# Yotsuei/ClearConverse

Hardware: AMD Instinct MI355X
Metric: xRT (audio-sec/wall-sec) end-to-end, 30 s 16 kHz clips (higher is better)
Workload: dtype bf16

## Files before the change

### clearconverse_amd/csrc/resnet.hip

```cpp
#include <string>
#include <vector>
#include <math.h>
#include "../../include/ccx.h"
#include "ccx_common.h"
#include "gemm_bf16.h"
#include "model_store.h"

namespace {

constexpr int FB_LEN = 400, FB_SHIFT = 160, FB_NFFT = 512, FB_MELS = 80, FB_MELW = 64;
constexpr int RN_C0 = 32, RN_EMB = 256, RN_STAGES = 4;
constexpr int RN_BLOCKS[RN_STAGES] = {3, 4, 6, 3};

__global__ __launch_bounds__(256) void fbank_kernel(const float* __restrict__ wav, long stride, int T, const float* __restrict__ window,
                                                    const float2* __restrict__ twiddle, const float* __restrict__ melw,
                                                    const int* __restrict__ mel_start, const int* __restrict__ mel_len,
                                                    float* __restrict__ feats_t) {
  __shared__ float2 buf[4][FB_NFFT];
  __shared__ float2 tw[FB_NFFT / 2];
  const int lane = threadIdx.x & 63, wave = threadIdx.x >> 6;
  for (int i = threadIdx.x; i < FB_NFFT / 2; i += 256) tw[i] = twiddle[i];
  const int chunk = blockIdx.y;
  const int t = blockIdx.x * 4 + wave;
  const bool live = t < T;
  const float* x = wav + (long)chunk * stride + (long)(live ? t : 0) * FB_SHIFT;
  float2* b = buf[wave];
  float v[7];
  float sm = 0.f;
#pragma unroll
  for (int j = 0; j < 7; j++) {
    const int i = lane + 64 * j;
    v[j] = i < FB_LEN ? x[i] * 32768.f : 0.f;
    sm += v[j];
  }
  const float mean = wave_reduce_sum(sm) / (float)FB_LEN;
#pragma unroll
  for (int j = 0; j < 7; j++) {
    const int i = lane + 64 * j;
    if (i < FB_LEN) b[i].y = v[j] - mean;
  }
  __syncthreads();
  float z[7];
#pragma unroll
  for (int j = 0; j < 7; j++) {
    const int i = lane + 64 * j;
    z[j] = 0.f;
    if (i < FB_LEN) z[j] = (b[i].y - 0.97f * b[i > 0 ? i - 1 : 0].y) * window[i];
  }
  __syncthreads();
#pragma unroll
  for (int j = 0; j < 8; j++) {
    const int i = lane + 64 * j;
    const int r = (int)(__brev((unsigned)i) >> 23);
    b[r] = make_float2(j < 7 ? z[j] : 0.f, 0.f);
  }
  __syncthreads();
  for (int s = 1; s <= 9; s++) {
    const int half = 1 << (s - 1);
#pragma unroll
    for (int q = 0; q < 4; q++) {
      const int bf = lane + 64 * q;
      const int grp = bf >> (s - 1), pos = bf & (half - 1);
      const int i0 = (grp << s) + pos, i1 = i0 + half;
      const float2 w = tw[pos << (9 - s)];
      const float2 a = b[i0], c = b[i1];
      const float2 m = make_float2(c.x * w.x - c.y * w.y, c.x * w.y + c.y * w.x);
      b[i0] = make_float2(a.x + m.x, a.y + m.y);
      b[i1] = make_float2(a.x - m.x, a.y - m.y);
    }
    __syncthreads();
  }
#pragma unroll
  for (int q = 0; q < 4; q++) {
    const int k = lane + 64 * q;
    const float2 c = b[k];
    b[k].x = c.x * c.x + c.y * c.y;
  }
  __syncthreads();
  for (int m = lane; m < FB_MELS; m += 64) {
    const int st = mel_start[m], ln = mel_len[m];
    float acc = 0.f;
    for (int k = 0; k < ln; k++) acc = fmaf(melw[m * FB_MELW + k], b[st + k].x, acc);
    if (live) feats_t[((long)chunk * FB_MELS + m) * T + t] = logf(fmaxf(acc, 1.1920929e-07f));
  }
}

__global__ __launch_bounds__(256) void fbank_mean_kernel(const float* __restrict__ feats_t, int T, float* __restrict__ mean) {
  __shared__ float sh[4];
  const float* p = feats_t + (long)blockIdx.x * T;
  float s = 0.f;
  for (int i = threadIdx.x; i < T; i += 256) s += p[i];
  s = wave_reduce_sum(s);
  if ((threadIdx.x & 63) == 0) sh[threadIdx.x >> 6] = s;
  __syncthreads();
  if (threadIdx.x == 0) mean[blockIdx.x] = (sh[0] + sh[1] + sh[2] + sh[3]) / (float)T;
}

__global__ __launch_bounds__(256) void conv1_kernel(const float* __restrict__ feats_t, const float* __restrict__ mean, int T,
                                                    const float* __restrict__ w, const float* __restrict__ bias,
                                                    bf16_t* __restrict__ out) {
  __shared__ float sw[RN_C0 * 9 + RN_C0];
  for (int i = threadIdx.x; i < RN_C0 * 9 + RN_C0; i += 256) sw[i] = i < RN_C0 * 9 ? w[i] : bias[i - RN_C0 * 9];
  __syncthreads();
  const int t = blockIdx.x * 256 + threadIdx.x;
  const int f = blockIdx.y, chunk = blockIdx.z;
  if (t >= T) return;
  float x[9];
#pragma unroll
  for (int kh = 0; kh < 3; kh++) {
    const int ff = f + kh - 1;
    const bool fin = ff >= 0 && ff < FB_MELS;
    const float mu = fin ? mean[chunk * FB_MELS + ff] : 0.f;
    const float* row = feats_t + ((long)chunk * FB_MELS + (fin ? ff : 0)) * T;
#pragma unroll
    for (int kw = 0; kw < 3; kw++) {
      const int tt = t + kw - 1;
      x[kh * 3 + kw] = (fin && tt >= 0 && tt < T) ? row[tt] - mu : 0.f;
    }
  }
  const long Wp = T + 2;
  bf16_t* dst = out + (((long)chunk * (FB_MELS + 2) + f + 1) * Wp + t + 1) * RN_C0;
#pragma unroll
  for (int c8 = 0; c8 < RN_C0 / 8; c8++) {
    float o[8];
#pragma unroll
    for (int j = 0; j < 8; j++) {
      const int c = c8 * 8 + j;
      float a = sw[RN_C0 * 9 + c];
#pragma unroll
      for (int k = 0; k < 9; k++) a = fmaf(sw[c * 9 + k], x[k], a);
      o[j] = fmaxf(a, 0.f);
    }
    uint4 pk;
    pk.x = pack_bf16x2(o[0], o[1]); pk.y = pack_bf16x2(o[2], o[3]); pk.z = pack_bf16x2(o[4], o[5]); pk.w = pack_bf16x2(o[6], o[7]);
    ((uint4*)dst)[c8] = pk;
  }
}

template <bool HAS_RESID>
__global__ __launch_bounds__(256) void conv3x3_c32_kernel(const bf16_t* __restrict__ in, const bf16_t* __restrict__ wpk,
                                                          const float* __restrict__ bias, const bf16_t* __restrict__ resid,
                                                          bf16_t* __restrict__ out, int H, int W) {
  constexpr int TW = 64, TH = 4, PITCH = 96;
  __shared__ __attribute__((aligned(16))) char tile[(TH + 2) * (TW + 2) * PITCH];
  const int tid = threadIdx.x, lane = tid & 63, wave = tid >> 6;
  const int l15 = lane & 15, hq = lane >> 4;
  const long Wp = W + 2;
  const int y0 = blockIdx.y * TH, img = blockIdx.z;
  const bf16_t* src = in + ((long)img * (H + 2) + y0) * Wp * 32;
  constexpr int NCH = (TH + 2) * (TW + 2) * 4, NIT = (NCH + 255) / 256;
  uint4 stg[NIT];
  uint4 rres[4];
  const long orow = ((long)img * (H + 2) + y0 + wave + 1) * Wp + 1;
  auto fetch = [&](int x0) {
#pragma unroll
    for (int it = 0; it < NIT; it++) {
      const int idx = tid + 256 * it;
      const int row = idx / ((TW + 2) * 4), rem = idx - row * (TW + 2) * 4;
      const int px = rem >> 2, q = rem & 3;
      stg[it] = make_uint4(0, 0, 0, 0);
      if (idx < NCH && x0 + px < Wp) stg[it] = *(const uint4*)(src + ((long)row * Wp + x0 + px) * 32 + q * 8);
    }
    if (HAS_RESID) {
#pragma unroll
      for (int pt = 0; pt < 4; pt++) {
        const int x = x0 + pt * 16 + l15;
        rres[pt] = make_uint4(0, 0, 0, 0);
        if (x < W) rres[pt] = *(const uint4*)(resid + (orow + x) * 32 + 8 * hq);
      }
    }
  };
  auto put = [&]() {
#pragma unroll
    for (int it = 0; it < NIT; it++) {
      const int idx = tid + 256 * it;
      const int row = idx / ((TW + 2) * 4), rem = idx - row * (TW + 2) * 4;
      const int px = rem >> 2, q = rem & 3;
      if (idx < NCH) *(uint4*)(tile + (row * (TW + 2) + px) * PITCH + q * 16) = stg[it];
    }
  };
  fetch(0);
  bf16x8 wf[9][2];
#pragma unroll
  for (int t = 0; t < 9; t++)
#pragma unroll
    for (int j = 0; j < 2; j++) {
      const int co = 8 * (l15 >> 2) + 4 * j + (l15 & 3);
      wf[t][j] = *(const bf16x8*)(wpk + (long)co * 384 + (t / 3) * 128 + (t % 3) * 32 + hq * 8);
    }
  float bv[8];
#pragma unroll
  for (int i = 0; i < 8; i++) bv[i] = bias[8 * hq + i];
  const int n_tiles = (W + TW - 1) / TW;
  for (int k = 0; k < n_tiles; k++) {
    const int x0 = k * TW;
    put();
    uint4 rcur[4];
    if (HAS_RESID) {
#pragma unroll
      for (int pt = 0; pt < 4; pt++) rcur[pt] = rres[pt];
    }
    __syncthreads();
    if (k + 1 < n_tiles) fetch(x0 + TW);
    f32x4 acc[4][2];
#pragma unroll
    for (int pt = 0; pt < 4; pt++)
#pragma unroll
      for (int j = 0; j < 2; j++) acc[pt][j] = (f32x4){0.f, 0.f, 0.f, 0.f};
#pragma unroll
    for (int t = 0; t < 9; t++) {
      const int kh = t / 3, kw = t % 3;
#pragma unroll
      for (int pt = 0; pt < 4; pt++) {
        const bf16x8 bfrag = *(const bf16x8*)(tile + ((wave + kh) * (TW + 2) + pt * 16 + l15 + kw) * PITCH + hq * 16);
#pragma unroll
        for (int j = 0; j < 2; j++) acc[pt][j] = __builtin_amdgcn_mfma_f32_16x16x32_bf16(wf[t][j], bfrag, acc[pt][j], 0, 0, 0);
      }
    }
#pragma unroll
    for (int pt = 0; pt < 4; pt++) {
      const int x = x0 + pt * 16 + l15;
      if (x >= W) continue;
      float v[8];
#pragma unroll
      for (int j = 0; j < 2; j++)
#pragma unroll
        for (int r = 0; r < 4; r++) v[4 * j + r] = acc[pt][j][r] + bv[4 * j + r];
      const long off = (orow + x) * 32 + 8 * hq;
      if (HAS_RESID) {
        const uint32_t rw[4] = {rcur[pt].x, rcur[pt].y, rcur[pt].z, rcur[pt].w};
#pragma unroll
        for (int i = 0; i < 4; i++) {
          v[2 * i] += __uint_as_float(rw[i] << 16);
          v[2 * i + 1] += __uint_as_float(rw[i] & 0xffff0000u);
        }
      }
      uint4 o;
      o.x = pack_bf16x2(fmaxf(v[0], 0.f), fmaxf(v[1], 0.f)); o.y = pack_bf16x2(fmaxf(v[2], 0.f), fmaxf(v[3], 0.f));
      o.z = pack_bf16x2(fmaxf(v[4], 0.f), fmaxf(v[5], 0.f)); o.w = pack_bf16x2(fmaxf(v[6], 0.f), fmaxf(v[7], 0.f));
      *(uint4*)(out + off) = o;
    }
    __syncthreads();
  }
}

__global__ __launch_bounds__(256) void tstp_kernel(const bf16_t* __restrict__ act, int W4, const int* __restrict__ mask_chunk,
                                                   const float* __restrict__ weights, int n_w, float* __restrict__ pooled) {
  const int h = blockIdx.x, j = blockIdx.y, c = threadIdx.x;
  const int chunk = mask_chunk ? mask_chunk[j] : j;
  const long Wp = W4 + 2;
  const bf16_t* base = act + (((long)chunk * 12 + h + 1) * Wp + 1) * 256 + c;
  const float* wj = weights ? weights + (long)j * n_w : nullptr;
  float v1 = 0.f, v2 = 0.f, sx = 0.f;
  const float scale = (float)n_w / (float)W4;
  for (int t = 0; t < W4; t++) {
    const float w = wj ? wj[min((int)floorf(t * scale), n_w - 1)] : 1.f;
    v1 += w; v2 += w * w;
    sx = fmaf(w, bf16_to_f32(base[(long)t * 256]), sx);
  }
  v1 += 1e-8f;
  const float mean = sx / v1;
  float sq = 0.f;
  for (int t = 0; t < W4; t++) {
    const float w = wj ? wj[min((int)floorf(t * scale), n_w - 1)] : 1.f;
    const float d = bf16_to_f32(base[(long)t * 256]) - mean;
    sq = fmaf(w, d * d, sq);
  }
  const float var = sq / (v1 - v2 / v1 + 1e-8f);
  float* o = pooled + (long)j * 5120;
  o[c * 10 + h] = mean;
  o[2560 + c * 10 + h] = sqrtf(var);
}

__global__ __launch_bounds__(256) void embed_linear_kernel(const float* __restrict__ pooled, const float* __restrict__ W,
                                                           const float* __restrict__ bias, float* __restrict__ out) {
  const int lane = threadIdx.x & 63, o = blockIdx.x * 4 + (threadIdx.x >> 6), j = blockIdx.y;
  const float4* p = (const float4*)(pooled + (long)j * 5120);
  const float4* w = (const float4*)(W + (long)o * 5120);
  float s = 0.f;
  for (int i = lane; i < 5120 / 4; i += 64) {
    const float4 a = p[i], b = w[i];
    s += a.x * b.x + a.y * b.y + a.z * b.z + a.w * b.w;
  }
  s = wave_reduce_sum(s);
  if (lane == 0) out[(long)j * RN_EMB + o] = s + bias[o];
}

struct Conv {
  bf16_t* W = nullptr;
  float* b = nullptr;
  int cin = 0, cout = 0, k = 3, stride = 1, Kpad = 0;
};
struct Block {
  Conv c1, c2, sc;
  bool has_sc = false;
};

}

struct ccx_resnet {
  ccx_ctx* ctx = nullptr;
  int max_chunks = 0, max_masks = 0, max_frames = 0;
  long max_samples = 0;
  bool finalized = false;
  ccx_dev_store store{"resnet"};
  float *window = nullptr, *melw = nullptr;
  float2* twiddle = nullptr;
  int *mel_start = nullptr, *mel_len = nullptr;
  float *c1w = nullptr, *c1b = nullptr, *segW = nullptr, *segb = nullptr;
  std::vector<Block> blocks;
  float *feats_t = nullptr, *fmean = nullptr, *pooled = nullptr;
  bf16_t* act[RN_STAGES][3] = {};
  size_t act_elems[RN_STAGES] = {};
  int* mask_chunk_dev = nullptr;
  std::vector<int> mask_host[4];
  int mask_slot = 0;
  int last_T = -1;
  int halo_chunks = 0;
};

namespace {

int bn_fold(ccx_resnet* r, const std::string& name, int c, std::vector<float>& scale, std::vector<float>& shift) {
  CCX_NEED(r->store, g, name + ".weight", c); CCX_NEED(r->store, be, name + ".bias", c);
  CCX_NEED(r->store, rm, name + ".running_mean", c); CCX_NEED(r->store, rv, name + ".running_var", c);
  scale.resize(c); shift.resize(c);
  for (int i = 0; i < c; i++) {
    scale[i] = g->data[i] / sqrtf(rv->data[i] + 1e-5f);
    shift[i] = be->data[i] - rm->data[i] * scale[i];
  }
  return CCX_OK;
}

int load_conv(ccx_resnet* r, const std::string& wname, const std::string& bnname, int cin, int cout, int k, int stride, Conv& cv) {
  CCX_NEED(r->store, w, wname, (int64_t)cout * cin * k * k);
  std::vector<float> sc, sh;
  CCX_TRY(bn_fold(r, bnname, cout, sc, sh));
  cv.cin = cin; cv.cout = cout; cv.k = k; cv.stride = stride;
  cv.Kpad = ccx_align(k * cin, 64);
  std::vector<bf16_t> packed((size_t)cout * k * cv.Kpad, 0);
  for (int o = 0; o < cout; o++)
    for (int c = 0; c < cin; c++)
      for (int kh = 0; kh < k; kh++)
        for (int kw = 0; kw < k; kw++)
          packed[((size_t)o * k + kh) * cv.Kpad + kw * cin + c] = ccx_host_f32_to_bf16(w->data[(((size_t)o * cin + c) * k + kh) * k + kw] * sc[o]);
  CCX_TRY(r->store.upload(&cv.W, packed));
  CCX_TRY(r->store.upload(&cv.b, sh));
  return CCX_OK;
}

__global__ __launch_bounds__(256) void halo_zero_kernel(bf16_t* b0, bf16_t* b1, bf16_t* b2, int c0, int H, long Wp, int C) {
  bf16_t* buf = blockIdx.z == 0 ? b0 : (blockIdx.z == 1 ? b1 : b2);
  const int y = blockIdx.x;
  bf16_t* row = buf + (((long)(c0 + blockIdx.y) * (H + 2) + y) * Wp) * C;
  const uint4 z = make_uint4(0, 0, 0, 0);
  if (y == 0 || y == H + 1) {
    const long n = Wp * C / 8;
    for (long i = threadIdx.x; i < n; i += 256) ((uint4*)row)[i] = z;
  } else {
    const int n = C / 8;
    for (int i = threadIdx.x; i < 2 * n; i += 256) {
      bf16_t* cell = i < n ? row : row + (Wp - 1) * C;
      ((uint4*)cell)[i < n ? i : i - n] = z;
    }
  }
}

struct StageDims { int H, W, C; long Wp; };
void stage_dims(int T, StageDims (&d)[RN_STAGES]) {
  int H = FB_MELS, W = T, C = RN_C0;
  for (int s = 0; s < RN_STAGES; s++) {
    d[s] = {H, W, C, (long)W + 2};
    H /= 2; W = (W - 1) / 2 + 1; C *= 2;
  }
}

int run_conv(ccx_resnet* r, const Conv& cv, int epi, const bf16_t* in, const StageDims& di, bf16_t* out, const StageDims& dn,
             const bf16_t* resid, int n_chunks, hipStream_t st) {
  if (cv.cin == 32 && cv.cout == 32 && cv.k == 3 && cv.stride == 1 && di.H % 4 == 0 && (epi == EPI_BF16_RELU || epi == EPI_BF16_ADD_RELU)) {
    const dim3 grid(1, di.H / 4, n_chunks);
    {
      ccx_prof_scope ps(r->ctx, st, "conv3x3_c32_kernel", 2.0 * 9 * 32 * 32 * (double)n_chunks * di.H * di.W,
                        (double)n_chunks * di.H * di.W * 64.0 * (resid ? 3 : 2));
      if (resid) hipLaunchKernelGGL(conv3x3_c32_kernel<true>, grid, dim3(256), 0, st, in, cv.W, cv.b, resid, out, di.H, di.W);
      else hipLaunchKernelGGL(conv3x3_c32_kernel<false>, grid, dim3(256), 0, st, in, cv.W, cv.b, resid, out, di.H, di.W);
    }
    CCX_CHECK_LAUNCH(r->ctx);
    return CCX_OK;
  }
  GemmParams p;
  memset(&p, 0, sizeof(p));
  const int s = cv.stride;
  const int RI = (di.H + 2) / s;
  p.A = in + (cv.k == 1 ? (di.Wp + 1) * di.C : 0);
  p.lda = (long)s * di.C;
  p.K = cv.Kpad; p.ntaps = cv.k; p.a_tap_stride = di.Wp * di.C;
  p.W = cv.W; p.ldw = (long)cv.k * cv.Kpad;
  p.M = (int)((long)n_chunks * RI * di.Wp); p.N = cv.cout;
  p.bias = cv.b; p.out = out; p.ldo = cv.cout;
  p.rpb_in = (int)di.Wp; p.rpb_valid = dn.W; p.rpb_out = (int)dn.Wp; p.roff = (int)dn.Wp + 1;
  p.img_rows_in = RI; p.img_rows_valid = dn.H; p.img_rows_out = dn.H + 2;
  p.resid_bf16 = resid; p.ldrb = cv.cout;
  return ccx_launch_gemm(r->ctx, epi, p, st);
}

}

extern "C" {

int ccx_resnet_create(ccx_ctx* ctx, int max_chunks, int64_t max_samples, int max_masks, ccx_resnet** out) {
  if (!ctx || !out) return CCX_ERR_ARG;
  CCX_REQUIRE(ctx, max_chunks >= 1 && max_masks >= 1 && max_samples >= FB_LEN + 7 * FB_SHIFT, "resnet_create: bad capacities");
  const int max_frames = 1 + (int)((max_samples - FB_LEN) / FB_SHIFT);
  CCX_REQUIRE(ctx, (long)max_chunks * 82 * (max_frames + 2) < (1L << 31), "resnet_create: max_chunks x frames too large for one launch");
  ccx_resnet* r = new ccx_resnet();
  r->ctx = ctx; r->store.ctx = ctx; r->max_chunks = max_chunks; r->max_masks = max_masks; r->max_samples = max_samples;
  r->max_frames = max_frames;
  *out = r;
  return CCX_OK;
}

void ccx_resnet_destroy(ccx_resnet* r) {
  if (!r) return;
  r->store.free_all();
  delete r;
}

int ccx_resnet_set_tensor(ccx_resnet* r, const char* name, const float* data, int64_t numel) {
  if (!r) return CCX_ERR_ARG;
  CCX_REQUIRE(r->ctx, !r->finalized && name && data && numel > 0, "resnet: set_tensor bad arguments");
  return r->store.stage(name, data, numel);
}

int ccx_resnet_finalize(ccx_resnet* r) {
  if (!r) return CCX_ERR_ARG;
  ccx_ctx* ctx = r->ctx;
  CCX_REQUIRE(ctx, !r->finalized, "resnet: finalize called twice");
  {
    std::vector<float> win(FB_LEN);
    for (int i = 0; i < FB_LEN; i++) win[i] = (float)(0.54 - 0.46 * cos(2.0 * M_PI * i / (FB_LEN - 1)));
    std::vector<float2> tw(FB_NFFT / 2);
    for (int i = 0; i < FB_NFFT / 2; i++) tw[i] = make_float2((float)cos(-2.0 * M_PI * i / FB_NFFT), (float)sin(-2.0 * M_PI * i / FB_NFFT));
    auto mel = [](double f) { return 1127.0 * log(1.0 + f / 700.0); };
    const double mlo = mel(20.0), mhi = mel(8000.0), delta = (mhi - mlo) / (FB_MELS + 1);
    std::vector<float> mw((size_t)FB_MELS * FB_MELW, 0.f);
    std::vector<int> ms(FB_MELS, 0), ml(FB_MELS, 0);
    for (int m = 0; m < FB_MELS; m++) {
      const double left = mlo + m * delta, center = left + delta, right = center + delta;
      int first = -1, last = -1;
      std::vector<float> wts(FB_NFFT / 2, 0.f);
      for (int k = 0; k < FB_NFFT / 2; k++) {
        const double mk = mel(16000.0 / FB_NFFT * k);
        const double up = (mk - left) / (center - left), down = (right - mk) / (right - center);
        const double wv = fmax(0.0, fmin(up, down));
        wts[k] = (float)wv;
        if (wv > 0.0) { if (first < 0) first = k; last = k; }
      }
      if (first < 0) { first = 0; last = -1; }
      CCX_REQUIRE(ctx, last - first + 1 <= FB_MELW, "resnet: mel filter %d spans %d bins", m, last - first + 1);
      ms[m] = first; ml[m] = last - first + 1;
      for (int k = first; k <= last; k++) mw[(size_t)m * FB_MELW + (k - first)] = wts[k];
    }
    CCX_TRY(r->store.upload(&r->window, win)); CCX_TRY(r->store.upload(&r->twiddle, tw)); CCX_TRY(r->store.upload(&r->melw, mw));
    CCX_TRY(r->store.upload(&r->mel_start, ms)); CCX_TRY(r->store.upload(&r->mel_len, ml));
  }
  {
    CCX_NEED(r->store, w, "resnet.conv1.weight", RN_C0 * 9);
    std::vector<float> sc, sh;
    CCX_TRY(bn_fold(r, "resnet.bn1", RN_C0, sc, sh));
    std::vector<float> wf(RN_C0 * 9);
    for (int c = 0; c < RN_C0; c++)
      for (int k = 0; k < 9; k++) wf[c * 9 + k] = w->data[c * 9 + k] * sc[c];
    CCX_TRY(r->store.upload(&r->c1w, wf)); CCX_TRY(r->store.upload(&r->c1b, sh));
  }
  int cin = RN_C0;
  for (int s = 0; s < RN_STAGES; s++) {
    const int cout = RN_C0 << s;
    for (int b = 0; b < RN_BLOCKS[s]; b++) {
      const std::string p = "resnet.layer" + std::to_string(s + 1) + "." + std::to_string(b) + ".";
      const int stride = (s > 0 && b == 0) ? 2 : 1;
      Block blk;
      CCX_TRY(load_conv(r, p + "conv1.weight", p + "bn1", cin, cout, 3, stride, blk.c1));
      CCX_TRY(load_conv(r, p + "conv2.weight", p + "bn2", cout, cout, 3, 1, blk.c2));
      blk.has_sc = stride != 1 || cin != cout;
      if (blk.has_sc) CCX_TRY(load_conv(r, p + "shortcut.0.weight", p + "shortcut.1", cin, cout, 1, stride, blk.sc));
      r->blocks.push_back(blk);
      cin = cout;
    }
  }
  {
    CCX_NEED(r->store, w, "resnet.seg_1.weight", (int64_t)RN_EMB * 5120); CCX_NEED(r->store, b, "resnet.seg_1.bias", RN_EMB);
    CCX_TRY(r->store.upload(&r->segW, w->data)); CCX_TRY(r->store.upload(&r->segb, b->data));
  }
  r->store.staged.clear();
  const int T = r->max_frames;
  CCX_TRY(r->store.alloc(&r->feats_t, (size_t)r->max_chunks * FB_MELS * T, true));
  CCX_TRY(r->store.alloc(&r->fmean, (size_t)r->max_chunks * FB_MELS, true));
  CCX_TRY(r->store.alloc(&r->pooled, (size_t)r->max_masks * 5120, true));
  CCX_TRY(r->store.alloc(&r->mask_chunk_dev, (size_t)r->max_masks, true));
  StageDims d[RN_STAGES];
  stage_dims(T, d);
  for (int s = 0; s < RN_STAGES; s++) {
    r->act_elems[s] = (size_t)r->max_chunks * (d[s].H + 2) * d[s].Wp * d[s].C + 4 * d[s].Wp * d[s].C + 1024;
    for (int k = 0; k < 3; k++) CCX_TRY(r->store.alloc(&r->act[s][k], r->act_elems[s], true));
  }
  r->finalized = true;
  return CCX_OK;
}

int ccx_resnet_embed(ccx_resnet* r, const float* wav_dev, int64_t stride, int n_samples, int n_chunks, const float* weights_dev,
                     int n_w, const int* mask_chunk, int n_masks, float* out_dev, void* stream_) {
  if (!r) return CCX_ERR_ARG;
  ccx_ctx* ctx = r->ctx;
  hipStream_t st = (hipStream_t)stream_;
  CCX_REQUIRE(ctx, r->finalized, "resnet: not finalized");
  CCX_REQUIRE(ctx, wav_dev && out_dev && n_chunks >= 1 && n_chunks <= r->max_chunks, "resnet_embed: bad chunk count %d (max %d)", n_chunks, r->max_chunks);
  CCX_REQUIRE(ctx, n_samples <= stride && n_samples <= r->max_samples, "resnet_embed: n_samples %d exceeds stride or capacity", n_samples);
  const int T = n_samples >= FB_LEN ? 1 + (n_samples - FB_LEN) / FB_SHIFT : 0;
  StageDims d[RN_STAGES];
  stage_dims(T > 0 ? T : 1, d);
  CCX_REQUIRE(ctx, T >= 1 && d[3].W >= 2, "resnet_embed: %d samples are too short (at least two pooled frames are needed)", n_samples);
  if (weights_dev) {
    CCX_REQUIRE(ctx, mask_chunk && n_masks >= 1 && n_masks <= r->max_masks && n_w >= 1, "resnet_embed: bad mask arguments");
    for (int j = 0; j < n_masks; j++)
      CCX_REQUIRE(ctx, mask_chunk[j] >= 0 && mask_chunk[j] < n_chunks, "resnet_embed: mask_chunk[%d]=%d out of range", j, mask_chunk[j]);
    std::vector<int>& keep = r->mask_host[r->mask_slot++ & 3];
    keep.assign(mask_chunk, mask_chunk + n_masks);
    CCX_HIP(ctx, hipMemcpyAsync(r->mask_chunk_dev, keep.data(), (size_t)n_masks * 4, hipMemcpyHostToDevice, st));
  } else {
    n_masks = n_chunks;
    CCX_REQUIRE(ctx, n_masks <= r->max_masks, "resnet_embed: %d chunks exceed the mask capacity %d", n_masks, r->max_masks);
  }
  if (T != r->last_T) { r->last_T = T; r->halo_chunks = 0; }
  if (n_chunks > r->halo_chunks) {
    for (int s = 0; s < RN_STAGES; s++)
      hipLaunchKernelGGL(halo_zero_kernel, dim3(d[s].H + 2, n_chunks - r->halo_chunks, 3), dim3(256), 0, st, r->act[s][0], r->act[s][1],
                         r->act[s][2], r->halo_chunks, d[s].H, d[s].Wp, d[s].C);
    CCX_CHECK_LAUNCH(ctx);
    r->halo_chunks = n_chunks;
  }
  {
    ccx_prof_scope ps(ctx, st, "fbank_kernel", 0.0, (double)n_chunks * n_samples * 4 + (double)n_chunks * T * FB_MELS * 4);
    hipLaunchKernelGGL(fbank_kernel, dim3(ccx_cdiv(T, 4), n_chunks), dim3(256), 0, st, wav_dev, (long)stride, T, r->window, r->twiddle,
                       r->melw, r->mel_start, r->mel_len, r->feats_t);
  }
  CCX_CHECK_LAUNCH(ctx);
  hipLaunchKernelGGL(fbank_mean_kernel, dim3(n_chunks * FB_MELS), dim3(256), 0, st, r->feats_t, T, r->fmean);
  CCX_CHECK_LAUNCH(ctx);
  {
    ccx_prof_scope ps(ctx, st, "conv1_kernel", 2.0 * 9 * RN_C0 * (double)n_chunks * FB_MELS * T,
                      (double)n_chunks * FB_MELS * T * (4 + RN_C0 * 2));
    hipLaunchKernelGGL(conv1_kernel, dim3(ccx_cdiv(T, 256), FB_MELS, n_chunks), dim3(256), 0, st, r->feats_t, r->fmean, T, r->c1w, r->c1b,
                       r->act[0][0]);
  }
  CCX_CHECK_LAUNCH(ctx);
  int bi = 0, cur = 0;
  const bf16_t* x = r->act[0][0];
  int xs = 0;
  for (int s = 0; s < RN_STAGES; s++) {
    for (int b = 0; b < RN_BLOCKS[s]; b++, bi++) {
      const Block& blk = r->blocks[bi];
      bf16_t* tbuf; bf16_t* ybuf; bf16_t* scbuf = nullptr;
      if (xs == s) {
        tbuf = r->act[s][(cur + 1) % 3]; ybuf = r->act[s][(cur + 2) % 3];
      } else {
        tbuf = r->act[s][0]; ybuf = r->act[s][1]; scbuf = r->act[s][2];
      }
      CCX_TRY(run_conv(r, blk.c1, EPI_BF16_RELU, x, d[xs], tbuf, d[s], nullptr, n_chunks, st));
      const bf16_t* resid = x;
      if (blk.has_sc) {
        CCX_REQUIRE(ctx, scbuf != nullptr, "resnet: shortcut convolution inside a stage");
        CCX_TRY(run_conv(r, blk.sc, EPI_BF16, x, d[xs], scbuf, d[s], nullptr, n_chunks, st));
        resid = scbuf;
      }
      CCX_TRY(run_conv(r, blk.c2, EPI_BF16_ADD_RELU, tbuf, d[s], ybuf, d[s], resid, n_chunks, st));
      x = ybuf; xs = s;
      cur = (int)(ybuf == r->act[s][0] ? 0 : (ybuf == r->act[s][1] ? 1 : 2));
    }
  }
  hipLaunchKernelGGL(tstp_kernel, dim3(10, n_masks), dim3(256), 0, st, x, d[3].W, weights_dev ? r->mask_chunk_dev : nullptr, weights_dev,
                     n_w, r->pooled);
  CCX_CHECK_LAUNCH(ctx);
  hipLaunchKernelGGL(embed_linear_kernel, dim3(RN_EMB / 4, n_masks), dim3(256), 0, st, r->pooled, r->segW, r->segb, out_dev);
  CCX_CHECK_LAUNCH(ctx);
  return CCX_OK;
}

}
```

Measured before the change: 1667.

## Add persistent direct 3x3 conv kernel for 64-channel ResNet stage

Adds a dedicated direct 3x3 convolution kernel for the stage-1 64-channel layers. It is persistent (one block per CU processing a contiguous range of tiles) and keeps all weights in registers. Input tiles are double-buffered into LDS with global_load_lds and an XOR swizzle, and the residual loads and epilogue stores are overlapped with MFMA work. This replaces the generic implicit-GEMM path for these layers to cut im2col-style overhead and improve overlap. It costs heavy hand-written asm, a large register footprint and a new env toggle. It only affects stage 1 of the ResNet, a part of the end-to-end pipeline.

```diff
diff --git a/clearconverse_amd/csrc/resnet.hip b/clearconverse_amd/csrc/resnet.hip
--- a/clearconverse_amd/csrc/resnet.hip
+++ b/clearconverse_amd/csrc/resnet.hip
@@ -242,6 +242,181 @@
     }
     __syncthreads();
   }
+}
+
+constexpr int C64_TW = 64, C64_TH = 4;
+constexpr int C64_NPIX = (C64_TH + 2) * (C64_TW + 2);
+constexpr int C64_NDMA = (C64_NPIX + 7) / 8;
+constexpr int C64_TILE = C64_NDMA * 1024;
+constexpr int C64_LDS = 2 * C64_TILE;
+
+template <bool HAS_RESID>
+__global__ __launch_bounds__(256, 1) void conv3x3_c64_kernel(const bf16_t* __restrict__ in, const bf16_t* __restrict__ wpk,
+                                                             const float* __restrict__ bias, const bf16_t* __restrict__ resid,
+                                                             bf16_t* __restrict__ out, int H, int W, int n_tiles, int total_tiles,
+                                                             int tiles_per_block) {
+  typedef const __attribute__((address_space(1))) void* gptr_t;
+  typedef __attribute__((address_space(3))) void* lptr_t;
+  constexpr int TW = C64_TW, TH = C64_TH;
+  extern __shared__ __attribute__((aligned(16))) char smem[];
+  const int tid = threadIdx.x, lane = tid & 63;
+  const int wave = __builtin_amdgcn_readfirstlane(tid >> 6);
+  const int l15 = lane & 15, hq = lane >> 4;
+  const int Wp = W + 2;
+  const int g0 = blockIdx.x * tiles_per_block;
+  const int g1 = g0 + tiles_per_block < total_tiles ? g0 + tiles_per_block : total_tiles;
+  if (g0 >= g1) return;
+  const int strips = H / TH;
+  auto locate = [&](int g, int& x0, long& prow) {
+    const int strip = g / n_tiles, k = g - strip * n_tiles;
+    const int img = strip / strips, ys = strip - img * strips;
+    x0 = k * TW;
+    prow = (long)img * (H + 2) + ys * TH;
+  };
+  constexpr int NII = (C64_NDMA + 3) / 4;
+  const int dchunk = ((lane & 7) ^ (lane >> 3)) * 8;
+  auto fetch = [&](int g, char* tile) {
+    int x0; long prow;
+    locate(g, x0, prow);
+    const bf16_t* src = in + prow * Wp * 64 + dchunk;
+#pragma unroll
+    for (int ii = 0; ii < NII; ii++) {
+      const int i = wave + 4 * ii;
+      if (i < C64_NDMA) {
+        int P = 8 * i + (lane >> 3);
+        P = P < C64_NPIX ? P : 0;
+        const int row = P / (TW + 2), px = P - row * (TW + 2);
+        const int gx = x0 + px < Wp ? x0 + px : 0;
+        asm volatile("s_mov_b32 m0, %0\n\ts_nop 0\n\tglobal_load_lds_dwordx4 %1, off"
+                     :: "s"(__builtin_amdgcn_readfirstlane((unsigned)(uintptr_t)(lptr_t)(tile + i * 1024))), "v"(src + (row * Wp + gx) * 64) : "memory", "m0");
+      }
+    }
+  };
+  fetch(g0, smem);
+  bf16x8 wf[9][2][4];
+#pragma unroll
+  for (int t = 0; t < 9; t++)
+#pragma unroll
+    for (int ks = 0; ks < 2; ks++)
+#pragma unroll
+      for (int j = 0; j < 4; j++) {
+        const int co = 32 * (j >> 1) + 8 * (l15 >> 2) + 4 * (j & 1) + (l15 & 3);
+        wf[t][ks][j] = *(const bf16x8*)(wpk + (long)co * 576 + (t / 3) * 192 + (t % 3) * 64 + ks * 32 + hq * 8);
+        if (t >= 3) asm volatile("" : "+a"(wf[t][ks][j]));
+        else asm volatile("" : "+v"(wf[t][ks][j]));
+      }
+  float bv[16];
+#pragma unroll
+  for (int j = 0; j < 4; j++)
+#pragma unroll
+    for (int r = 0; r < 4; r++) bv[4 * j + r] = bias[32 * (j >> 1) + 8 * hq + 4 * (j & 1) + r];
+#pragma unroll
+  for (int i = 0; i < 16; i++) asm volatile("" ::"v"(bv[i]));
+  int boff[9];
+#pragma unroll
+  for (int t = 0; t < 9; t++) {
+    const int P = (wave + t / 3) * (TW + 2) + (t % 3) + l15;
+    boff[t] = P * 128 + ((hq ^ (P & 7)) << 4);
+  }
+  f32x4 acc[2][4];
+#pragma unroll
+  for (int j = 0; j < 4; j++) acc[1][j] = (f32x4){0.f, 0.f, 0.f, 0.f};
+  uint4 pres[2] = {make_uint4(0, 0, 0, 0), make_uint4(0, 0, 0, 0)};
+  bf16_t* pdst = out;
+  bool pvalid = false;
+  uint32_t pk[8];
+  auto epi_step = [&](int s, const f32x4 (&a)[4]) {
+    if (s < 8) {
+      float e[2];
+#pragma unroll
+      for (int q = 0; q < 2; q++) {
+        const int c = 2 * s + q;
+        e[q] = a[c >> 2][c & 3] + bv[c];
+      }
+      if (HAS_RESID) {
+        const uint4& rq = pres[s >> 2];
+        const uint32_t rw = (s & 3) == 0 ? rq.x : (s & 3) == 1 ? rq.y : (s & 3) == 2 ? rq.z : rq.w;
+        e[0] += __uint_as_float(rw << 16);
+        e[1] += __uint_as_float(rw & 0xffff0000u);
+      }
+      pk[s] = pack_bf16x2(fmaxf(e[0], 0.f), fmaxf(e[1], 0.f));
+      asm volatile("" : "+v"(pk[s]));
+    } else if (s < 10) {
+      const int i = s - 8;
+      if (pvalid) *(uint4*)(pdst + 32 * i) = make_uint4(pk[4 * i], pk[4 * i + 1], pk[4 * i + 2], pk[4 * i + 3]);
+    }
+  };
+  uint4 rres[4][2];
+  auto request_resid = [&](int pt, int x0, long orow) {
+    const int x = x0 + pt * 16 + l15;
+    const bf16_t* rp = resid + (orow + (x < W ? x : 0)) * 64 + 8 * hq;
+    asm volatile("global_load_dwordx4 %0, %1, off" : "=&v"(rres[pt][0]) : "v"(rp) : "memory");
+    asm volatile("global_load_dwordx4 %0, %1, off offset:64" : "=&v"(rres[pt][1]) : "v"(rp) : "memory");
+  };
+  if (HAS_RESID) {
+    int x0; long prow;
+    locate(g0, x0, prow);
+#pragma unroll
+    for (int pt = 0; pt < 4; pt++) request_resid(pt, x0, (prow + wave + 1) * Wp + 1);
+  }
+  asm volatile("s_waitcnt vmcnt(0)" ::: "memory");
+  __syncthreads();
+  for (int g = g0; g < g1; g++) {
+    const char* tile = smem + ((g - g0) & 1) * C64_TILE;
+    int x0; long prow;
+    locate(g, x0, prow);
+    const long orow = (prow + wave + 1) * Wp + 1;
+    const int gn = g + 1 < g1 ? g + 1 : g;
+    int nx0; long nprow;
+    locate(gn, nx0, nprow);
+    const long norow = (nprow + wave + 1) * Wp + 1;
+    fetch(gn, smem + ((g - g0 + 1) & 1) * C64_TILE);
+    constexpr int RD = 4;
+    auto bread = [&](int n) {
+      const int pt = n / 18, t = (n % 18) >> 1, ks = n & 1;
+      return *(const bf16x8*)(tile + pt * 2048 + (boff[t] ^ (ks * 64)));
+    };
+    bf16x8 ring[RD];
+#pragma unroll
+    for (int n = 0; n < RD; n++) ring[n] = bread(n);
+    __builtin_amdgcn_sched_barrier(0);
+#pragma unroll
+    for (int pt = 0; pt < 4; pt++) {
+      f32x4 (&A)[4] = acc[pt & 1];
+#pragma unroll
+      for (int s = 0; s < 18; s++) {
+        const int n = pt * 18 + s, t = s >> 1, ks = s & 1;
+        const bf16x8 bfrag = ring[n % RD];
+        if (n + RD < 72) ring[n % RD] = bread(n + RD);
+#pragma unroll
+        for (int j = 0; j < 4; j++)
+          A[j] = __builtin_amdgcn_mfma_f32_16x16x32_bf16(wf[t][ks][j], bfrag, s == 0 ? (f32x4){0.f, 0.f, 0.f, 0.f} : A[j], 0, 0, 0);
+        epi_step(s, acc[(pt & 1) ^ 1]);
+        __builtin_amdgcn_sched_barrier(0);
+      }
+      const int x = x0 + pt * 16 + l15;
+      pvalid = x < W;
+      pdst = out + (orow + x) * 64 + 8 * hq;
+      if (HAS_RESID) {
+        asm volatile("s_waitcnt vmcnt(18)" ::: "memory");
+#pragma unroll
+        for (int i = 0; i < 2; i++) {
+          asm volatile("v_mov_b32 %0, %1" : "=v"(pres[i].x) : "v"(rres[pt][i].x));
+          asm volatile("v_mov_b32 %0, %1" : "=v"(pres[i].y) : "v"(rres[pt][i].y));
+          asm volatile("v_mov_b32 %0, %1" : "=v"(pres[i].z) : "v"(rres[pt][i].z));
+          asm volatile("v_mov_b32 %0, %1" : "=v"(pres[i].w) : "v"(rres[pt][i].w));
+        }
+        request_resid(pt, nx0, norow);
+      }
+      __builtin_amdgcn_sched_barrier(0);
+    }
+    if (HAS_RESID) asm volatile("s_waitcnt vmcnt(8)" ::: "memory");
+    else asm volatile("s_waitcnt vmcnt(2)" ::: "memory");
+    __syncthreads();
+  }
+#pragma unroll
+  for (int s = 0; s < 10; s++) epi_step(s, acc[1]);
+  asm volatile("s_waitcnt vmcnt(0)" ::: "memory");
 }
 
 __global__ __launch_bounds__(256) void tstp_kernel(const bf16_t* __restrict__ act, int W4, const int* __restrict__ mask_chunk,
@@ -317,6 +492,7 @@
   int mask_slot = 0;
   int last_T = -1;
   int halo_chunks = 0;
+  int n_cu = 0;
 };
 
 namespace {
@@ -376,7 +552,7 @@
 }
 
 int run_conv(ccx_resnet* r, const Conv& cv, int epi, const bf16_t* in, const StageDims& di, bf16_t* out, const StageDims& dn,
-             const bf16_t* resid, int n_chunks, hipStream_t st) {
+             const bf16_t* resid, int n_chunks, bool direct, hipStream_t st) {
   if (cv.cin == 32 && cv.cout == 32 && cv.k == 3 && cv.stride == 1 && di.H % 4 == 0 && (epi == EPI_BF16_RELU || epi == EPI_BF16_ADD_RELU)) {
     const dim3 grid(1, di.H / 4, n_chunks);
     {
@@ -384,6 +560,24 @@
                         (double)n_chunks * di.H * di.W * 64.0 * (resid ? 3 : 2));
       if (resid) hipLaunchKernelGGL(conv3x3_c32_kernel<true>, grid, dim3(256), 0, st, in, cv.W, cv.b, resid, out, di.H, di.W);
       else hipLaunchKernelGGL(conv3x3_c32_kernel<false>, grid, dim3(256), 0, st, in, cv.W, cv.b, resid, out, di.H, di.W);
+    }
+    CCX_CHECK_LAUNCH(r->ctx);
+    return CCX_OK;
+  }
+  if (direct && cv.cin == 64 && cv.cout == 64 && cv.k == 3 && cv.stride == 1 && di.H % C64_TH == 0 &&
+      (epi == EPI_BF16_RELU || epi == EPI_BF16_ADD_RELU)) {
+    const int n_tiles = ccx_cdiv(di.W, C64_TW);
+    const long total = (long)n_chunks * (di.H / C64_TH) * n_tiles;
+    const int tpb = (int)((total + r->n_cu - 1) / r->n_cu);
+    const dim3 grid((unsigned)((total + tpb - 1) / tpb));
+    static ccx_lds_optin optin_r, optin_n;
+    CCX_HIP(r->ctx, optin_r.ensure(r->ctx->device, (const void*)conv3x3_c64_kernel<true>, C64_LDS));
+    CCX_HIP(r->ctx, optin_n.ensure(r->ctx->device, (const void*)conv3x3_c64_kernel<false>, C64_LDS));
+    {
+      ccx_prof_scope ps(r->ctx, st, "conv3x3_c64_kernel", 2.0 * 9 * 64 * 64 * (double)n_chunks * di.H * di.W,
+                        (double)n_chunks * di.H * di.W * 128.0 * (resid ? 3 : 2));
+      if (resid) hipLaunchKernelGGL(conv3x3_c64_kernel<true>, grid, dim3(256), C64_LDS, st, in, cv.W, cv.b, resid, out, di.H, di.W, n_tiles, (int)total, tpb);
+      else hipLaunchKernelGGL(conv3x3_c64_kernel<false>, grid, dim3(256), C64_LDS, st, in, cv.W, cv.b, resid, out, di.H, di.W, n_tiles, (int)total, tpb);
     }
     CCX_CHECK_LAUNCH(r->ctx);
     return CCX_OK;
@@ -416,6 +610,7 @@
   ccx_resnet* r = new ccx_resnet();
   r->ctx = ctx; r->store.ctx = ctx; r->max_chunks = max_chunks; r->max_masks = max_masks; r->max_samples = max_samples;
   r->max_frames = max_frames;
+  if (hipDeviceGetAttribute(&r->n_cu, hipDeviceAttributeMultiprocessorCount, ctx->device) != hipSuccess || r->n_cu < 1) r->n_cu = 256;
   *out = r;
   return CCX_OK;
 }
@@ -554,6 +749,8 @@
                        r->act[0][0]);
   }
   CCX_CHECK_LAUNCH(ctx);
+  const char* denv = getenv("CCX_RESNET_DIRECT");
+  const bool direct = denv ? atoi(denv) != 0 : true;
   int bi = 0, cur = 0;
   const bf16_t* x = r->act[0][0];
   int xs = 0;
@@ -566,14 +763,14 @@
       } else {
         tbuf = r->act[s][0]; ybuf = r->act[s][1]; scbuf = r->act[s][2];
       }
-      CCX_TRY(run_conv(r, blk.c1, EPI_BF16_RELU, x, d[xs], tbuf, d[s], nullptr, n_chunks, st));
+      CCX_TRY(run_conv(r, blk.c1, EPI_BF16_RELU, x, d[xs], tbuf, d[s], nullptr, n_chunks, direct, st));
       const bf16_t* resid = x;
       if (blk.has_sc) {
         CCX_REQUIRE(ctx, scbuf != nullptr, "resnet: shortcut convolution inside a stage");
-        CCX_TRY(run_conv(r, blk.sc, EPI_BF16, x, d[xs], scbuf, d[s], nullptr, n_chunks, st));
+        CCX_TRY(run_conv(r, blk.sc, EPI_BF16, x, d[xs], scbuf, d[s], nullptr, n_chunks, direct, st));
         resid = scbuf;
       }
-      CCX_TRY(run_conv(r, blk.c2, EPI_BF16_ADD_RELU, tbuf, d[s], ybuf, d[s], resid, n_chunks, st));
+      CCX_TRY(run_conv(r, blk.c2, EPI_BF16_ADD_RELU, tbuf, d[s], ybuf, d[s], resid, n_chunks, direct, st));
       x = ybuf; xs = s;
       cur = (int)(ybuf == r->act[s][0] ? 0 : (ybuf == r->act[s][1] ? 1 : 2));
     }
```

New measurement: 1670, median of 5. About the same (+0.2%).
